# MarkTakken/kf2vecFSW

Measured on AMD Instinct MI355X. Metric: Gbases/s k-mer→.kf build at k=7; achieved HBM GB/s vs gfx950 peak, higher is better.
Workload: dtype u32

## Files before the change

kf2vecfsw_amd/counter.py:

```python
from __future__ import annotations

import ctypes
import dataclasses
import os
from typing import Sequence

import numpy as np
import torch

from . import _native as N

ALIGN = 16


def num_bins(k: int) -> int:
    return int(N.lib().kf_num_bins(k))


def tables(k: int) -> tuple[np.ndarray, np.ndarray]:
    nb = num_bins(k)
    code2col = np.empty(1 << (2 * k), dtype=np.uint32)
    col2rep = np.empty(nb, dtype=np.uint32)
    n = ctypes.c_uint64(0)
    N.check(N.lib().kf_tables(k, code2col.ctypes.data, col2rep.ctypes.data, ctypes.byref(n)), "kf_tables")
    assert n.value == nb
    return code2col, col2rep


def vocab_text(k: int) -> bytes:
    nb = num_bins(k)
    buf = np.empty(nb * (k + 1), dtype=np.uint8)
    w = ctypes.c_uint64(0)
    N.check(N.lib().kf_vocab_text(k, buf.ctypes.data, buf.size, ctypes.byref(w)), "kf_vocab_text")
    return buf[: w.value].tobytes()


def index_records(data: np.ndarray, fmt: int = N.KF_FMT_AUTO, base: int = 0) -> tuple[np.ndarray, int]:
    data = np.ascontiguousarray(data, dtype=np.uint8)
    cap = 64
    while True:
        out = np.empty(2 * cap, dtype=np.uint64)
        n = ctypes.c_uint64(0)
        f = ctypes.c_int(0)
        rc = N.lib().kf_index_records(data.ctypes.data, data.size, fmt, base, out.ctypes.data, cap,
                                      ctypes.byref(n), ctypes.byref(f))
        if rc == N.KF_ERANGE:
            cap = int(n.value)
            continue
        N.check(rc, "kf_index_records")
        return out[: 2 * n.value], int(f.value)


@dataclasses.dataclass
class HostBatch:
    data: torch.Tensor | None
    off: np.ndarray
    excl: np.ndarray | None
    names: list[str]
    dev_data: torch.Tensor | None = None
    dev_event: object = None
    fastq: bool = False

    @property
    def n(self) -> int:
        return len(self.off) - 1

    def seq_chars(self) -> int:
        d = self.data.numpy()
        nl = int(np.count_nonzero(d[: int(self.off[-1])] == 10))
        excl = self.excl if self.excl is not None else np.concatenate(
            [index_records(d[int(self.off[i]): int(self.off[i + 1])],
                           N.KF_FMT_FASTQ if self.fastq else N.KF_FMT_FASTA, int(self.off[i]))[0]
             for i in range(self.n)] or [np.zeros(0, np.uint64)])
        ex = int((excl[1::2] - excl[0::2]).sum()) if excl.size else 0
        return int(self.off[-1] - self.off[0]) - nl - ex


def _layout(sizes: Sequence[int]) -> np.ndarray:
    off = np.zeros(len(sizes) + 1, dtype=np.uint64)
    pos = 0
    for i, s in enumerate(sizes):
        off[i] = pos
        pos += (int(s) + ALIGN - 1) // ALIGN * ALIGN
    off[-1] = pos
    return off


def _alloc_host(nbytes: int, pin: bool) -> torch.Tensor:
    pin = pin and torch.cuda.is_available()
    return torch.empty(max(nbytes, ALIGN), dtype=torch.uint8, pin_memory=pin)


def pack_genomes(blobs: Sequence[bytes | np.ndarray], names: Sequence[str] | None = None,
                 fmt: int = N.KF_FMT_AUTO, pin: bool = True) -> HostBatch:
    sizes = [len(b) for b in blobs]
    off = _layout(sizes)
    data = _alloc_host(int(off[-1]), pin)
    d = data.numpy()
    d[: int(off[-1])] = 10
    excl = []
    for i, b in enumerate(blobs):
        a = np.frombuffer(b, dtype=np.uint8) if isinstance(b, (bytes, bytearray, memoryview)) else np.asarray(b, np.uint8)
        lo = int(off[i])
        d[lo: lo + a.size] = a
        iv, _ = index_records(d[lo: lo + a.size], fmt, lo)
        excl.append(iv)
    ex = np.concatenate(excl) if excl else np.zeros(0, np.uint64)
    return HostBatch(data, off, ex.astype(np.uint64), list(names) if names else [str(i) for i in range(len(blobs))])


def pack_files(paths: Sequence[str], names: Sequence[str] | None = None, fmt: int = N.KF_FMT_AUTO,
               pin: bool = True, threads: int = 8, pool=None, times: dict | None = None,
               buf: torch.Tensor | None = None, index: bool = True, piece: int = 1 << 20) -> HostBatch:
    from concurrent.futures import ThreadPoolExecutor
    import time
    t0 = time.perf_counter()
    sizes = [os.path.getsize(p) for p in paths]
    off = _layout(sizes)
    if buf is not None and buf.numel() >= max(int(off[-1]), ALIGN):
        data = buf[: max(int(off[-1]), ALIGN)]
    else:
        data = _alloc_host(int(off[-1]), pin)
    d = data.numpy()
    if times is not None:
        times["alloc_ms"] = round((time.perf_counter() - t0) * 1e3, 3)
    nthr = getattr(pool, "_max_workers", None) or max(1, int(threads))
    if paths:
        enc = [os.fsencode(p) for p in paths]
        arr = (ctypes.c_char_p * len(enc))(*enc)
        sz = np.asarray(sizes, dtype=np.uint64)
        N.check(N.lib().kf_read_files(arr, len(enc), sz.ctypes.data, off.ctypes.data, d.ctypes.data,
                                      int(piece), int(nthr)), "kf_read_files")

    def is_fastq(i: int) -> bool:
        return fmt == N.KF_FMT_FASTQ or (fmt == N.KF_FMT_AUTO and sizes[i] > 0 and d[int(off[i])] == ord("@"))

    def on_host(i: int) -> bool:
        return index or is_fastq(i)

    def host_index(i: int):
        lo, sz = int(off[i]), sizes[i]
        return index_records(d[lo: lo + sz], fmt, lo)[0] if on_host(i) else None

    if not any(on_host(i) for i in range(len(paths))):
        return HostBatch(data, off, None, list(names) if names else list(paths))
    if not index and all(is_fastq(i) or sizes[i] == 0 for i in range(len(paths))):
        return HostBatch(data, off, None, list(names) if names else list(paths), fastq=True)
    if pool is not None:
        excl = list(pool.map(host_index, range(len(paths))))
    elif threads > 1 and len(paths) > 1:
        with ThreadPoolExecutor(max_workers=min(threads, len(paths))) as ex:
            excl = list(ex.map(host_index, range(len(paths))))
    else:
        excl = [host_index(i) for i in range(len(paths))]
    if not index and all(e is None for e in excl):
        return HostBatch(data, off, None, list(names) if names else list(paths))
    excl = [e if e is not None else index_records(d[int(off[i]): int(off[i]) + sizes[i]], N.KF_FMT_FASTA,
                                                  int(off[i]))[0] for i, e in enumerate(excl)]
    ex = np.concatenate(excl) if excl else np.zeros(0, np.uint64)
    return HostBatch(data, off, ex.astype(np.uint64), list(names) if names else list(paths))


def pack_ranges(ranges: Sequence[tuple[str, int, int]], names: Sequence[str] | None = None, pin: bool = True,
                threads: int = 8, chunk: int = 64 << 20, index: bool = False, buf: torch.Tensor | None = None,
                fastq: bool = False) -> HostBatch:
    from concurrent.futures import ThreadPoolExecutor
    sizes = [e - a for _, a, e in ranges]
    off = _layout(sizes)
    if buf is not None and buf.numel() >= max(int(off[-1]), ALIGN):
        data = buf[: max(int(off[-1]), ALIGN)]
    else:
        data = _alloc_host(int(off[-1]), pin)
    d = data.numpy()
    for i, sz in enumerate(sizes):
        d[int(off[i]) + sz: int(off[i + 1])] = 10
    jobs = []
    for i, (p, a, e) in enumerate(ranges):
        for x in range(a, e, chunk):
            jobs.append((p, x, min(e, x + chunk), int(off[i]) + x - a))

    def read(job):
        p, x, y, dst = job
        fd = os.open(p, os.O_RDONLY)
        try:
            got = 0
            mv = memoryview(d[dst: dst + (y - x)])
            while got < y - x:
                r = os.preadv(fd, [mv[got:]], x + got)
                if r <= 0:
                    raise N.NativeError(f"short read on {p}")
                got += r
        finally:
            os.close(fd)

    with ThreadPoolExecutor(max_workers=max(1, int(threads))) as ex:
        list(ex.map(read, jobs))
        excl = None
        if index and not fastq:
            parts = list(ex.map(lambda i: index_records(d[int(off[i]): int(off[i]) + sizes[i]], N.KF_FMT_FASTA,
                                                        int(off[i]))[0], range(len(ranges))))
            excl = (np.concatenate(parts) if parts else np.zeros(0, np.uint64)).astype(np.uint64)
    return HostBatch(data, off, excl, list(names) if names else [f"{p}:{a}" for p, a, _ in ranges], fastq=fastq)


@dataclasses.dataclass
class DeviceBatch:
    data: torch.Tensor
    off: torch.Tensor
    excl: torch.Tensor
    n: int
    n_excl: int
    irregular: tuple = ()


def index_on_device(data: torch.Tensor, off: torch.Tensor, n: int, nbytes: int) -> tuple[torch.Tensor, int]:
    dev = data.device
    s = _stream_ptr(dev)
    nb = (nbytes + 4095) // 4096
    scratch = torch.empty(nb + 1, dtype=torch.int32, device=dev)
    npairs = torch.zeros(1, dtype=torch.int64, device=dev)
    cap = 64 * n + 4096
    while True:
        excl = torch.empty(max(2 * cap, 2), dtype=torch.int64, device=dev)
        N.check(N.lib().kf_index_fasta(data.data_ptr(), off.data_ptr(), n, nbytes, excl.data_ptr(), cap,
                                       npairs.data_ptr(), scratch.data_ptr(), nb + 1, s), "kf_index_fasta")
        m = int(npairs.item())
        if m <= cap:
            return excl[: 2 * m], m
        cap = m


def index_fastq_on_device(data: torch.Tensor, off: torch.Tensor, n: int, nbytes: int, status_out: list | None = None
                          ) -> tuple[torch.Tensor, int, bool]:
    dev = data.device
    s = _stream_ptr(dev)
    L = N.lib()
    cap_lines = nbytes // 32 + 4 * n + 4096
    cap_pairs = nbytes // 128 + 2 * n + 4096
    info = torch.empty(2 + (n + 1) // 2, dtype=torch.int64, device=dev)
    while True:
        need = int(L.kf_index_fastq_scratch_bytes(nbytes, n, cap_lines))
        scratch = torch.empty(max(need // 8, 1), dtype=torch.int64, device=dev)
        excl = torch.empty(max(2 * cap_pairs, 2), dtype=torch.int64, device=dev)
        N.check(L.kf_index_fastq(data.data_ptr(), off.data_ptr(), n, nbytes, excl.data_ptr(), cap_pairs, cap_lines,
                                 info.data_ptr(), info.data_ptr() + 16, scratch.data_ptr(), need, s), "kf_index_fastq")
        h = info.cpu().numpy()
        m, lines = int(h[0]), int(h[1])
        if lines > cap_lines:
            cap_lines, cap_pairs = lines, max(cap_pairs, lines // 4 + 2 * n + 1)
            continue
        if m > cap_pairs:
            cap_pairs = m
            continue
        status = h[2:].view(np.uint32)[:n]
        if (status == 2).any():
            raise N.NativeError("kf_index_fastq: genome offsets must be non-decreasing and end at or below the batch")
        if status_out is not None:
            status_out.append(status.copy())
        return excl[: 2 * m], m, not status.any()


INDEX_PATHS = {"fasta_device": 0, "fastq_device": 0, "fastq_host_fallback": 0}


def to_device(hb: HostBatch, device: torch.device | str = "cuda", fallback: bool = True) -> DeviceBatch:
    dev = torch.device(device)
    if hb.dev_data is not None:
        cur = torch.cuda.current_stream(dev)
        if hb.dev_event is not None:
            cur.wait_event(hb.dev_event)
        data = hb.dev_data
        data.record_stream(cur)
    else:
        data = hb.data.to(dev, non_blocking=True)
    if hb.excl is None:
        pin = hb.data is None or hb.data.is_pinned()
        off = torch.from_numpy(hb.off.view(np.int64))
        off = (off.pin_memory() if pin else off).to(dev, non_blocking=pin)
        nbytes = int(hb.off[-1])
        with torch.cuda.device(dev):
            if not hb.fastq:
                excl, m = index_on_device(data, off, hb.n, nbytes)
                INDEX_PATHS["fasta_device"] += 1
            else:
                st: list = []
                excl, m, regular = index_fastq_on_device(data, off, hb.n, nbytes, st)
                INDEX_PATHS["fastq_device" if regular or not fallback else "fastq_host_fallback"] += 1
                if not regular and not fallback:
                    return DeviceBatch(data, off, excl if m else torch.zeros(2, dtype=torch.int64, device=dev), hb.n, m,
                                       tuple(int(g) for g in np.flatnonzero(st[0])))
                if not regular:
                    d = data[:nbytes].cpu().numpy()
                    iv = np.concatenate([index_records(d[int(hb.off[i]): int(hb.off[i + 1])], N.KF_FMT_FASTQ,
                                                       int(hb.off[i]))[0] for i in range(hb.n)])
                    m = iv.size // 2
                    excl = torch.from_numpy(iv.view(np.int64)).to(dev)
        return DeviceBatch(data, off, excl if m else torch.zeros(2, dtype=torch.int64, device=dev), hb.n, m)
    ex = hb.excl if hb.excl.size else np.zeros(2, np.uint64)
    pin = hb.data is None or hb.data.is_pinned()
    n_off = (hb.off.size + 1) & ~1
    host = np.zeros(n_off + ex.size, np.int64)
    host[: hb.off.size] = hb.off.view(np.int64)
    host[n_off:] = ex.view(np.int64)
    small = torch.from_numpy(host)
    if pin:
        small = small.pin_memory()
    small = small.to(dev, non_blocking=pin)
    off, excl = small[: hb.off.size], small[n_off:]
    return DeviceBatch(data, off, excl, hb.n, hb.excl.size // 2)


def _stream_ptr(device: torch.device) -> int:
    return torch.cuda.current_stream(device).cuda_stream


def accumulate_rows(src: torch.Tensor, src_totals: torch.Tensor, seg: torch.Tensor, dst: torch.Tensor,
                    dst_totals: torch.Tensor, status: torch.Tensor, accumulate: bool = False,
                    stream: int | None = None) -> None:
    assert src.dtype == torch.int32 and dst.dtype == torch.int32 and src.is_contiguous() and dst.is_contiguous()
    assert src.dim() == 2 and dst.dim() == 2 and src.shape[1] == dst.shape[1]
    assert src_totals.dtype == torch.int64 and src_totals.shape == (src.shape[0],) and src_totals.is_contiguous()
    assert dst_totals.dtype == torch.int64 and dst_totals.shape == (dst.shape[0],) and dst_totals.is_contiguous()
    assert seg.dtype == torch.int32 and seg.shape == (dst.shape[0] + 1,) and seg.is_contiguous()
    assert status.dtype == torch.int32 and status.shape == (dst.shape[0],) and status.is_contiguous()
    s = _stream_ptr(dst.device) if stream is None else stream
    with torch.cuda.device(dst.device):
        N.check(N.lib().kf_rows_accumulate(src.data_ptr(), src_totals.data_ptr(), src.shape[0], seg.data_ptr(),
                                           dst.shape[0], dst.shape[1], dst.data_ptr(), dst_totals.data_ptr(),
                                           status.data_ptr(), N.KF_ACCUMULATE if accumulate else 0, s),
                "kf_rows_accumulate")


_DEV_TABLES: dict = {}


class KmerCounter:

    def __init__(self, k: int, device: torch.device | str = "cuda"):
        if not (N.KF_MIN_K <= k <= N.KF_MAX_K):
            raise ValueError(f"k={k} out of range [{N.KF_MIN_K}, {N.KF_MAX_K}]")
        self.k = k
        self.device = torch.device(device)
        if self.device.type != "cuda" or not torch.cuda.is_available():
            raise N.NativeError("KmerCounter needs a ROCm GPU (no CPU fallback)")
        self.nbins = num_bins(k)
        key = (k, self.device.index if self.device.index is not None else torch.cuda.current_device())
        if key not in _DEV_TABLES:
            c2c, c2r = tables(k)
            _DEV_TABLES[key] = (torch.from_numpy(c2c.view(np.int32)).to(self.device),
                                torch.from_numpy(c2r.view(np.int32)).to(self.device))
        self.code2col, self.col2rep = _DEV_TABLES[key]

    def launch_info(self) -> tuple[int, int, int]:
        g, b, l = ctypes.c_int(), ctypes.c_int(), ctypes.c_int()
        with torch.cuda.device(self.device):
            N.check(N.lib().kf_count_launch_info(self.k, ctypes.byref(g), ctypes.byref(b), ctypes.byref(l)),
                    "kf_count_launch_info")
        return g.value, b.value, l.value

    def reserve(self, max_genomes: int) -> None:
        with torch.cuda.device(self.device):
            N.check(N.lib().kf_workspace_reserve(self.k, int(max_genomes)), "kf_workspace_reserve")

    def alloc_out(self, n: int) -> tuple[torch.Tensor, torch.Tensor]:
        return (torch.empty((n, self.nbins), dtype=torch.int32, device=self.device),
                torch.empty(n, dtype=torch.int64, device=self.device))

    def count(self, db: DeviceBatch, counts: torch.Tensor | None = None, totals: torch.Tensor | None = None,
              accumulate: bool = False, stream: int | None = None) -> tuple[torch.Tensor, torch.Tensor]:
        if counts is None or totals is None:
            counts, totals = self.alloc_out(db.n)
        assert counts.shape == (db.n, self.nbins) and counts.dtype == torch.int32 and counts.is_contiguous()
        assert totals.shape == (db.n,) and totals.dtype == torch.int64
        assert db.data.data_ptr() % 16 == 0
        s = _stream_ptr(self.device) if stream is None else stream
        with torch.cuda.device(self.device):
            N.check(N.lib().kf_count_batch(
                db.data.data_ptr(), db.off.data_ptr(), db.n, db.excl.data_ptr() if db.n_excl else None,
                db.n_excl, self.code2col.data_ptr(), self.col2rep.data_ptr(), self.k,
                counts.data_ptr(), totals.data_ptr(), N.KF_ACCUMULATE if accumulate else 0, s), "kf_count_batch")
        return counts, totals


class SparseCounter:

    def __init__(self, k: int, device: torch.device | str = "cuda"):
        if not (N.KF_MIN_K <= k <= N.KF_SPARSE_MAX_K):
            raise ValueError(f"k={k} out of range [{N.KF_MIN_K}, {N.KF_SPARSE_MAX_K}]")
        self.k = k
        self.device = torch.device(device)
        if self.device.type != "cuda" or not torch.cuda.is_available():
            raise N.NativeError("SparseCounter needs a ROCm GPU (no CPU fallback)")
        self._work = None

    def workspace_bytes(self, batch_bytes: int, n: int) -> int:
        return int(N.lib().kf_sparse_workspace_bytes(self.k, int(batch_bytes), int(n)))

    def count(self, db: DeviceBatch, batch_bytes: int):
        batch_bytes = int(batch_bytes)
        need = self.workspace_bytes(batch_bytes, db.n)
        if self._work is None or self._work.numel() < need:
            self._work = None
            self._work = torch.empty(max(need, 256), dtype=torch.uint8, device=self.device)
        keys = torch.empty(max(batch_bytes, 1), dtype=torch.int64, device=self.device)
        counts = torch.empty(max(batch_bytes, 1), dtype=torch.int32, device=self.device)
        nuniq = torch.zeros(max(db.n, 1), dtype=torch.int64, device=self.device)
        s = _stream_ptr(self.device)
        with torch.cuda.device(self.device):
            N.check(N.lib().kf_sparse_count(
                db.data.data_ptr(), db.off.data_ptr(), db.n, batch_bytes,
                db.excl.data_ptr() if db.n_excl else None, db.n_excl, self.k,
                self._work.data_ptr(), self._work.numel(), keys.data_ptr(), counts.data_ptr(),
                nuniq.data_ptr(), s), "kf_sparse_count")
        return keys, counts, nuniq[: db.n]

    @staticmethod
    def nuniq_to_host(nuniq: torch.Tensor) -> np.ndarray:
        nu = nuniq.cpu().numpy()
        if nu.size and (nu == -1).any():
            raise N.NativeError("kf_sparse_count: genome offsets must be non-decreasing and end at or below "
                                "batch_bytes (nothing was counted)")
        if nu.size and (nu == -2).any():
            raise N.NativeError("kf_sparse_count: the sorted keys failed the device's order check")
        return nu

    def to_host(self, keys: torch.Tensor, counts: torch.Tensor, nuniq: torch.Tensor,
                off: np.ndarray) -> list[tuple[np.ndarray, np.ndarray]]:
        nu = self.nuniq_to_host(nuniq)
        if nu.size == 0 or int(nu.sum()) == 0:
            return [(np.zeros(0, np.uint64), np.zeros(0, np.uint32)) for _ in range(nu.size)]
        idx = torch.cat([torch.arange(int(off[g]), int(off[g]) + int(nu[g]), device=keys.device)
                         for g in range(nu.size)])
        hk = keys[idx].cpu().numpy().view(np.uint64)
        hc = counts[idx].cpu().numpy().view(np.uint32)
        out, pos = [], 0
        for g in range(nu.size):
            m = int(nu[g])
            out.append((hk[pos: pos + m], hc[pos: pos + m]))
            pos += m
        return out


def merge_tile() -> int:
    return int(N.lib().kf_sparse_merge_tile())


def merge_scratch_bytes(n_a: int, n_b: int) -> int:
    return int(N.lib().kf_sparse_merge_scratch_bytes(int(n_a), int(n_b)))


def merge_sorted(keys_a: torch.Tensor, counts_a: torch.Tensor, keys_b: torch.Tensor, counts_b: torch.Tensor,
                 stream: int | None = None):
    for k_, c_ in ((keys_a, counts_a), (keys_b, counts_b)):
        assert k_.dtype == torch.int64 and k_.dim() == 1 and k_.is_contiguous()
        assert c_.dtype in (torch.int32, torch.int64) and c_.shape == k_.shape and c_.is_contiguous()
        assert k_.device == keys_a.device and c_.device == keys_a.device
    dev = keys_a.device
    n_a, n_b = keys_a.numel(), keys_b.numel()
    keys = torch.empty(max(n_a + n_b, 1), dtype=torch.int64, device=dev)
    counts = torch.empty(max(n_a + n_b, 1), dtype=torch.int64, device=dev)
    n_out = torch.empty(1, dtype=torch.int64, device=dev)
    status = torch.empty(1, dtype=torch.int32, device=dev)
    need = merge_scratch_bytes(n_a, n_b)
    scratch = torch.empty(max(need // 8, 1), dtype=torch.int64, device=dev)
    s = _stream_ptr(dev) if stream is None else stream
    with torch.cuda.device(dev):
        N.check(N.lib().kf_sparse_merge(
            keys_a.data_ptr() if n_a else None, counts_a.data_ptr() if n_a else None,
            4 if counts_a.dtype == torch.int32 else 8, n_a,
            keys_b.data_ptr() if n_b else None, counts_b.data_ptr() if n_b else None,
            4 if counts_b.dtype == torch.int32 else 8, n_b,
            keys.data_ptr(), counts.data_ptr(), n_out.data_ptr(), status.data_ptr(), scratch.data_ptr(),
            8 * scratch.numel(), s), "kf_sparse_merge")
    return keys[: n_a + n_b], counts[: n_a + n_b], n_out, status


def merged_to_host(n_out: torch.Tensor, status: torch.Tensor) -> int:
    n, st = torch.cat([n_out, status.to(torch.int64)]).cpu().tolist()
    if st != 0:
        raise N.NativeError("kf_sparse_merge: an input list is not strictly ascending (nothing was merged)")
    return int(n)


def counts_to_numpy(counts: torch.Tensor) -> np.ndarray:
    return counts.cpu().numpy().view(np.uint32)


def features(counts: torch.Tensor, pseudocount: bool = False, raw_cnt: bool = False,
             scaler: float = 1.0) -> torch.Tensor:
    c = counts.to(torch.int64)
    c = torch.where(c < 0, c + (1 << 32), c)
    v = c.to(torch.float64)
    if pseudocount:
        v = v + 0.5
    if not raw_cnt:
        v = v / v.sum(dim=1, keepdim=True)
    return v * scaler if scaler != 1.0 else v


def chunk_features(counts: torch.Tensor, lo, n, scaler: float = 1.0, cap: int | None = None,
                   dtype: torch.dtype = torch.float32, out: torch.Tensor | None = None,
                   stream: int | None = None) -> torch.Tensor:
    assert counts.dtype in (torch.int16, torch.int32) and counts.dim() == 2 and counts.is_contiguous()
    assert dtype in (torch.float32, torch.float64)
    dev = counts.device
    if isinstance(lo, torch.Tensor) and lo.is_cuda:
        assert isinstance(n, torch.Tensor) and n.device == lo.device == dev and lo.shape == n.shape
        assert lo.dtype == n.dtype == torch.int64 and lo.is_contiguous() and n.is_contiguous()
        d_lo, d_n = lo, n
    else:
        def as_i64(x):
            x = np.asarray(x.cpu() if isinstance(x, torch.Tensor) else x)
            return x.view(np.int64) if x.dtype == np.uint64 else x.astype(np.int64)
        t = torch.from_numpy(np.stack([as_i64(lo).reshape(-1), as_i64(n).reshape(-1)]))
        d_lo, d_n = (t.pin_memory() if t.numel() else t).to(dev, non_blocking=True)
    ns, nbins = d_lo.numel(), counts.shape[1]
    if out is None:
        out = torch.empty((ns, nbins), dtype=dtype, device=dev)
    assert out.dtype == dtype and out.shape == (ns, nbins) and out.is_contiguous() and out.device == dev
    if ns == 0:
        return out
    status = torch.empty(1, dtype=torch.int32, device=dev)
    need = int(N.lib().kf_chunk_features_scratch_bytes(ns))
    work = torch.empty(need // 8, dtype=torch.int64, device=dev)
    s = _stream_ptr(dev) if stream is None else stream
    with torch.cuda.device(dev):
        N.check(N.lib().kf_chunk_features(
            counts.data_ptr() if counts.shape[0] else None, counts.element_size(), counts.shape[0], nbins,
            d_lo.data_ptr(), d_n.data_ptr(), ns, 0xFFFFFFFF if cap is None else int(cap), float(scaler),
# ... 220 lines not shown
```

kf2vecfsw_amd/csrc/kf_compact.h:

```cpp
#pragma once
#include "kf_scan.h"

namespace kf {
namespace {

constexpr int kCompactBlock = 256;
constexpr int kCompactPer = 16;
constexpr uint32_t kCompactSpan = kCompactBlock * kCompactPer;

__device__ __forceinline__ uint64_t compact_p0() {
    return (uint64_t)blockIdx.x * kCompactSpan + (uint64_t)threadIdx.x * kCompactPer;
}

template <typename T>
__device__ __forceinline__ void compact_count(uint32_t c, T* blk) {
    __shared__ uint32_t red[kCompactBlock / 64];
    const uint32_t all = block_sum<kCompactBlock / 64>(c, red);
    if (threadIdx.x == 0) blk[blockIdx.x] = all;
}

__device__ __forceinline__ uint64_t compact_first_slot(uint64_t base, uint32_t c) {
    __shared__ uint32_t wsum[kCompactBlock / 64];
    return base + block_excl_scan<kCompactBlock / 64>(c, wsum);
}

__global__ void __launch_bounds__(1024) compact_scan_kernel(uint32_t* blk, uint32_t nb, uint64_t* total64) {
    const uint32_t all = scan_with_carry(
        nb, [&](uint32_t i) { return blk[i]; }, [&](uint32_t i, uint32_t p) { blk[i] = p; });
    if (threadIdx.x == 0) {
        blk[nb] = all;
        if (total64) *total64 = all;
    }
}

}
}
```

kf2vecfsw_amd/csrc/kf_index.hip:

```cpp
#include <hip/hip_runtime.h>
#include <stdint.h>

#include "kf_compact.h"
#include "kf_internal.h"

namespace kf {
namespace {

constexpr int kIBlock = kCompactBlock;
constexpr int kIPer = kCompactPer;
constexpr uint32_t kISpan = kCompactSpan;

__device__ __forceinline__ uint32_t thread_heads(const uint8_t* bytes, uint64_t end, const uint64_t* goff, int n,
                                                 uint64_t p0) {
    uint32_t m = 0;
    if (p0 >= end) return 0;
    uint8_t prev = p0 > 0 ? bytes[p0 - 1] : (uint8_t)'\n';
    for (int q = 0; q < kIPer; ++q) {
        const uint64_t i = p0 + q;
        if (i >= end) break;
        const uint8_t c = bytes[i];
        if (c == '>') {
            bool start = prev == '\n' || i == 0;
            if (!start) {
                start = goff[last_at_or_before(n, i, [&](int g) { return goff[g]; })] == i;
            }
            if (start) m |= 1u << q;
        }
        prev = c;
    }
    return m;
}

__global__ void __launch_bounds__(kIBlock) idx_count_kernel(const uint8_t* bytes, uint64_t end, const uint64_t* goff,
                                                            int n, uint32_t* blk) {
    compact_count((uint32_t)__builtin_popcount(thread_heads(bytes, end, goff, n, compact_p0())), blk);
}

__global__ void __launch_bounds__(kIBlock) idx_scatter_kernel(const uint8_t* bytes, uint64_t end, const uint64_t* goff,
                                                              int n, const uint32_t* blk, uint64_t* excl,
                                                              uint64_t cap) {
    const uint64_t p0 = compact_p0();
    uint32_t m = thread_heads(bytes, end, goff, n, p0);
    uint64_t u = compact_first_slot(blk[blockIdx.x], (uint32_t)__builtin_popcount(m));
    while (m) {
        const int q = __builtin_ctz(m);
        m &= m - 1;
        const uint64_t j = p0 + (uint64_t)q;
        if (u < cap) {
            const uint64_t ge = goff[last_at_or_before(n, j, [&](int g) { return goff[g]; }) + 1];
            uint64_t e = j;
            while (e < ge && bytes[e] != '\n') ++e;
            excl[2 * u] = j;
            excl[2 * u + 1] = e;
        }
        ++u;
    }
}

constexpr uint32_t kQLevel = kScanLevel;
constexpr uint64_t kQMaxEntries = kScanMaxEntries;
constexpr auto fq_scan_level_kernel = scan_level_kernel<uint64_t>;

struct FqLayout {
    uint64_t nb, nb1, nb2;
    uint64_t ng1, ng2;
    uint64_t blk, blk1, blk2, g_nl, g_lines, g_end, g_pairs, g_pairs1, g_pairs2, nlpos, words;
};

inline uint64_t div_up(uint64_t a, uint64_t b) { return (a + b - 1) / b; }

inline FqLayout fq_layout(uint64_t batch_bytes, uint64_t n_genomes, uint64_t cap_lines) {
    FqLayout L;
    L.nb = div_up(batch_bytes, kISpan);
    L.nb1 = div_up(L.nb, kQLevel);
    L.nb2 = div_up(L.nb1, kQLevel);
    L.ng1 = div_up(n_genomes, kQLevel);
    L.ng2 = div_up(L.ng1, kQLevel);
    uint64_t w = 0;
    L.blk = w, w += L.nb;
    L.blk1 = w, w += L.nb1;
    L.blk2 = w, w += L.nb2;
    L.g_nl = w, w += n_genomes;
    L.g_lines = w, w += n_genomes;
    L.g_end = w, w += n_genomes;
    L.g_pairs = w, w += n_genomes;
    L.g_pairs1 = w, w += L.ng1;
    L.g_pairs2 = w, w += L.ng2;
    L.nlpos = w, w += cap_lines;
    L.words = w;
    return L;
}

__device__ __forceinline__ uint32_t nl_bits(uint32_t w) {
    const uint32_t x = w ^ 0x0A0A0A0Au;
    const uint32_t z = ~(((x & 0x7F7F7F7Fu) + 0x7F7F7F7Fu) | x | 0x7F7F7F7Fu);
    return (((z >> 7) * 0x00204081u) >> 21) & 0xFu;
}

__device__ __forceinline__ uint32_t thread_newlines(const uint8_t* bytes, uint64_t end, uint64_t p0) {
    if (p0 >= end) return 0;
    const uint4 v = *reinterpret_cast<const uint4*>(bytes + p0);
    uint32_t m = nl_bits(v.x) | nl_bits(v.y) << 4 | nl_bits(v.z) << 8 | nl_bits(v.w) << 12;
    if (end - p0 < kIPer) m &= (1u << (uint32_t)(end - p0)) - 1u;
    return m;
}

__global__ void __launch_bounds__(kIBlock) fq_count_kernel(const uint8_t* bytes, uint64_t end, uint64_t* blk) {
    compact_count((uint32_t)__builtin_popcount(thread_newlines(bytes, end, compact_p0())), blk);
}

__global__ void __launch_bounds__(kIBlock) fq_scatter_kernel(const uint8_t* bytes, uint64_t end, const uint64_t* blk,
                                                             const uint64_t* blk1, const uint64_t* blk2,
                                                             uint64_t* nlpos, uint64_t cap_lines) {
    const uint64_t p0 = compact_p0();
    uint32_t m = thread_newlines(bytes, end, p0);
    uint64_t u = compact_first_slot(scanned(blk, blk1, blk2, blockIdx.x), (uint32_t)__builtin_popcount(m));
    while (m) {
        const int q = __builtin_ctz(m);
        m &= m - 1;
        if (u < cap_lines) nlpos[u] = p0 + (uint64_t)q;
        ++u;
    }
}

__device__ __forceinline__ uint64_t first_at_or_after(const uint64_t* pos, uint64_t n, uint64_t x) {
    uint64_t lo = 0, hi = n;
    while (lo < hi) {
        const uint64_t mid = lo + ((hi - lo) >> 1);
        if (pos[mid] < x) lo = mid + 1;
        else hi = mid;
    }
    return lo;
}

__global__ void __launch_bounds__(kIBlock) fq_genome_kernel(const uint64_t* goff, int n, uint64_t end,
                                                            const uint64_t* nlpos, const uint64_t* n_lines,
                                                            uint64_t cap_lines, uint64_t* g_nl, uint64_t* g_lines,
                                                            uint64_t* g_end, uint64_t* g_pairs, uint32_t* status) {
    const uint64_t g = (uint64_t)blockIdx.x * kIBlock + threadIdx.x;
    if (g >= (uint64_t)n) return;
    const uint64_t tot = *n_lines, a = goff[g], b = goff[g + 1];
    uint64_t first = 0, lines = 0, cend = a;
    if (tot <= cap_lines) {
        if (b < a || b > end) {
            status[g] = 2;
        } else {
            first = first_at_or_after(nlpos, tot, a);
            const uint64_t last = first_at_or_after(nlpos, tot, b);
            uint64_t lo = first, hi = last;
            while (lo < hi) {
                const uint64_t mid = lo + ((hi - lo) >> 1);
                if (nlpos[mid] + (last - mid) == b) hi = mid;
                else lo = mid + 1;
            }
            cend = b - (last - lo);
            if (cend > a) lines = (lo - first) + 1;
        }
    }
    g_nl[g] = first;
    g_lines[g] = lines;
    g_end[g] = cend;
    g_pairs[g] = lines ? 1 + (lines + 1) / 4 : 0;
}

__global__ void __launch_bounds__(kIBlock) fq_pair_kernel(const uint8_t* bytes, const uint64_t* goff, int n,
                                                          const uint64_t* nlpos, const uint64_t* n_lines,
                                                          uint64_t cap_lines, const uint64_t* g_nl,
                                                          const uint64_t* g_lines, const uint64_t* g_end,
                                                          const uint64_t* g_pairs, const uint64_t* g_pairs1,
                                                          const uint64_t* g_pairs2, const uint64_t* n_pairs,
                                                          uint64_t* excl, uint64_t cap_pairs, uint32_t* status) {
    const uint64_t q = (uint64_t)blockIdx.x * kIBlock + threadIdx.x;
    if (q >= cap_pairs || q >= *n_pairs || *n_lines > cap_lines) return;
    const uint64_t g = (uint64_t)last_at_or_before(
        n, q, [&](int m) { return scanned(g_pairs, g_pairs1, g_pairs2, (uint64_t)m); });
    const uint64_t r = q - scanned(g_pairs, g_pairs1, g_pairs2, g);
    const uint64_t lines = g_lines[g], a = goff[g], cend = g_end[g];
    const uint64_t* nl = nlpos + g_nl[g];
    if (lines == 0 || r >= 1 + (lines + 1) / 4) return;
    auto start_of = [&](uint64_t j) { return j == 0 ? a : nl[j - 1] + 1; };
    auto end_of = [&](uint64_t j) { return j + 1 < lines ? nl[j] : cend; };
    uint64_t s, e;
    if (r == 0) {
        s = a;
        e = end_of(0);
    } else {
        const uint64_t plus = 4 * r - 2, to = plus + 2 < lines ? plus + 2 : lines - 1;
        s = start_of(plus);
        e = end_of(to);
    }
    excl[2 * q] = s;
    excl[2 * q + 1] = e;
    const uint64_t j0 = 4 * r;
    if (j0 >= lines) return;
    bool bad;
    uint64_t len_seq = 0;
    {
        const uint64_t s0 = start_of(j0), e0 = end_of(j0);
        bad = !(e0 > s0 && bytes[s0] == '@');
    }
    if (j0 + 1 < lines) {
        const uint64_t s1 = start_of(j0 + 1);
        len_seq = end_of(j0 + 1) - s1;
        bad |= len_seq > 0 && bytes[s1] == '+';
    }
    if (j0 + 2 < lines) {
        const uint64_t s2 = start_of(j0 + 2);
        bad |= !(end_of(j0 + 2) > s2 && bytes[s2] == '+');
    }
    if (j0 + 3 < lines) {
        const uint64_t len_qual = end_of(j0 + 3) - start_of(j0 + 3);
        bad |= len_seq == 0 ? len_qual != 0 : len_qual < len_seq;
    }
    if (bad) status[g] = 1;
}

}
}

using namespace kf;

extern "C" int kf_index_fasta(const uint8_t* d_bytes, const uint64_t* d_goff, int32_t n_genomes, uint64_t batch_bytes,
                              uint64_t* d_excl, uint64_t cap_pairs, uint64_t* d_n_pairs, uint32_t* d_scratch,
                              uint64_t scratch_words, void* stream) {
    if (n_genomes < 0) return kf_fail(KF_EINVAL, "n_genomes < 0");
    if (!d_n_pairs) return kf_fail(KF_EINVAL, "null device pointer");
    hipStream_t s = (hipStream_t)stream;
    if (n_genomes == 0 || batch_bytes == 0) {
        if (hipMemsetAsync(d_n_pairs, 0, 8, s) != hipSuccess) return kf_fail(KF_EHIP, "memset failed");
        return KF_OK;
    }
    if (!d_bytes || !d_goff || !d_scratch || (cap_pairs && !d_excl)) return kf_fail(KF_EINVAL, "null device pointer");
    const uint64_t nb = (batch_bytes + kISpan - 1) / kISpan;
    if (nb >= (1ull << 31)) return kf_fail(KF_EINVAL, "batch too large");
    if (scratch_words < nb + 1)
        return kf_fail(KF_ERANGE, "scratch needs %llu words", (unsigned long long)(nb + 1));
    hipLaunchKernelGGL(idx_count_kernel, dim3((uint32_t)nb), dim3(kIBlock), 0, s, d_bytes, batch_bytes, d_goff,
                       n_genomes, d_scratch);
    hipLaunchKernelGGL(compact_scan_kernel, dim3(1), dim3(1024), 0, s, d_scratch, (uint32_t)nb, d_n_pairs);
    hipLaunchKernelGGL(idx_scatter_kernel, dim3((uint32_t)nb), dim3(kIBlock), 0, s, d_bytes, batch_bytes, d_goff,
                       n_genomes, d_scratch, d_excl, cap_pairs);
    if (hipGetLastError() != hipSuccess) return kf_fail(KF_EHIP, "record index launch failed");
    return KF_OK;
}

extern "C" uint64_t kf_index_fastq_scratch_bytes(uint64_t batch_bytes, int32_t n_genomes, uint64_t cap_lines) {
    if (n_genomes < 0) return 0;
    return 8 * fq_layout(batch_bytes, (uint64_t)n_genomes, cap_lines).words;
}

extern "C" int kf_index_fastq(const uint8_t* d_bytes, const uint64_t* d_goff, int32_t n_genomes, uint64_t batch_bytes,
                              uint64_t* d_excl, uint64_t cap_pairs, uint64_t cap_lines, uint64_t* d_n,
                              uint32_t* d_status, void* d_scratch, uint64_t scratch_bytes, void* stream) {
    if (n_genomes < 0) return kf_fail(KF_EINVAL, "n_genomes < 0");
    if (!d_n) return kf_fail(KF_EINVAL, "null device pointer (d_n)");
    if (n_genomes > 0 && !d_status) return kf_fail(KF_EINVAL, "null device pointer (d_status)");
    hipStream_t s = (hipStream_t)stream;
    if (n_genomes == 0 || batch_bytes == 0) {
        if (hipMemsetAsync(d_n, 0, 16, s) != hipSuccess ||
            (n_genomes && hipMemsetAsync(d_status, 0, 4 * (size_t)n_genomes, s) != hipSuccess))
            return kf_fail(KF_EHIP, "memset failed");
        return KF_OK;
    }
    if (!d_bytes || !d_goff || !d_scratch || (cap_pairs && !d_excl)) return kf_fail(KF_EINVAL, "null device pointer");
    if (((uintptr_t)d_bytes & 15) || ((uintptr_t)d_scratch & 7))
        return kf_fail(KF_EINVAL, "d_bytes must be 16-byte and d_scratch 8-byte aligned");
    const FqLayout L = fq_layout(batch_bytes, (uint64_t)n_genomes, cap_lines);
    if (L.nb > kQMaxEntries) return kf_fail(KF_EINVAL, "batch too large");
    if ((uint64_t)n_genomes > kQMaxEntries) return kf_fail(KF_EINVAL, "too many genomes");
    if (cap_pairs >= (1ull << 31) * kIBlock) return kf_fail(KF_EINVAL, "cap_pairs too large");
    if (scratch_bytes < 8 * L.words)
        return kf_fail(KF_ERANGE, "scratch needs %llu bytes", (unsigned long long)(8 * L.words));
    uint64_t* w = (uint64_t*)d_scratch;
    if (hipMemsetAsync(d_status, 0, 4 * (size_t)n_genomes, s) != hipSuccess) return kf_fail(KF_EHIP, "memset failed");
    hipLaunchKernelGGL(fq_count_kernel, dim3((uint32_t)L.nb), dim3(kIBlock), 0, s, d_bytes, batch_bytes, w + L.blk);
    hipLaunchKernelGGL(fq_scan_level_kernel, dim3((uint32_t)L.nb1), dim3(kQLevel), 0, s, w + L.blk, L.nb, w + L.blk1);
    hipLaunchKernelGGL(fq_scan_level_kernel, dim3((uint32_t)L.nb2), dim3(kQLevel), 0, s, w + L.blk1, L.nb1,
                       w + L.blk2);
    hipLaunchKernelGGL(fq_scan_level_kernel, dim3(1), dim3(kQLevel), 0, s, w + L.blk2, L.nb2, d_n + 1);
    hipLaunchKernelGGL(fq_scatter_kernel, dim3((uint32_t)L.nb), dim3(kIBlock), 0, s, d_bytes, batch_bytes, w + L.blk,
                       w + L.blk1, w + L.blk2, w + L.nlpos, cap_lines);
    const uint32_t gb = (uint32_t)div_up((uint64_t)n_genomes, kIBlock);
    hipLaunchKernelGGL(fq_genome_kernel, dim3(gb), dim3(kIBlock), 0, s, d_goff, n_genomes, batch_bytes, w + L.nlpos,
                       d_n + 1, cap_lines, w + L.g_nl, w + L.g_lines, w + L.g_end, w + L.g_pairs, d_status);
    hipLaunchKernelGGL(fq_scan_level_kernel, dim3((uint32_t)L.ng1), dim3(kQLevel), 0, s, w + L.g_pairs,
                       (uint64_t)n_genomes, w + L.g_pairs1);
    hipLaunchKernelGGL(fq_scan_level_kernel, dim3((uint32_t)L.ng2), dim3(kQLevel), 0, s, w + L.g_pairs1, L.ng1,
                       w + L.g_pairs2);
    hipLaunchKernelGGL(fq_scan_level_kernel, dim3(1), dim3(kQLevel), 0, s, w + L.g_pairs2, L.ng2, d_n);
    if (cap_pairs)
        hipLaunchKernelGGL(fq_pair_kernel, dim3((uint32_t)div_up(cap_pairs, kIBlock)), dim3(kIBlock), 0, s, d_bytes,
                           d_goff, n_genomes, w + L.nlpos, d_n + 1, cap_lines, w + L.g_nl, w + L.g_lines, w + L.g_end,
                           w + L.g_pairs, w + L.g_pairs1, w + L.g_pairs2, d_n, d_excl, cap_pairs, d_status);
    if (hipGetLastError() != hipSuccess) return kf_fail(KF_EHIP, "FASTQ index launch failed");
    return KF_OK;
}
```

kf2vecfsw_amd/csrc/kf_scan.h:

```cpp
#pragma once
#include <hip/hip_runtime.h>
#include <stdint.h>

namespace kf {

typedef __attribute__((address_space(3))) uint32_t lds_u32;
__device__ __forceinline__ void lds_add(uint32_t a, uint32_t v) {
    __hip_atomic_fetch_add((lds_u32*)(uintptr_t)a, v, __ATOMIC_RELAXED, __HIP_MEMORY_SCOPE_WORKGROUP);
}
__device__ __forceinline__ uint32_t lds_add_rtn(uint32_t a, uint32_t v) {
    return __hip_atomic_fetch_add((lds_u32*)(uintptr_t)a, v, __ATOMIC_RELAXED, __HIP_MEMORY_SCOPE_WORKGROUP);
}

__device__ __forceinline__ void lds_barrier() { asm volatile("s_waitcnt lgkmcnt(0)\n\ts_barrier" ::: "memory"); }

__device__ __forceinline__ uint32_t wave_incl_scan(uint32_t v) {
    v += (uint32_t)__builtin_amdgcn_update_dpp(0, (int)v, 0x111, 0xF, 0xF, false);
    v += (uint32_t)__builtin_amdgcn_update_dpp(0, (int)v, 0x112, 0xF, 0xF, false);
    v += (uint32_t)__builtin_amdgcn_update_dpp(0, (int)v, 0x114, 0xF, 0xF, false);
    v += (uint32_t)__builtin_amdgcn_update_dpp(0, (int)v, 0x118, 0xF, 0xF, false);
    v += (uint32_t)__builtin_amdgcn_update_dpp(0, (int)v, 0x142, 0xA, 0xF, false);
    v += (uint32_t)__builtin_amdgcn_update_dpp(0, (int)v, 0x143, 0xC, 0xF, false);
    return v;
}
__device__ __forceinline__ uint64_t wave_incl_scan(uint64_t v) {
    const int lane = threadIdx.x & 63;
    for (int d = 1; d < 64; d <<= 1) {
        const uint64_t o = __shfl_up((unsigned long long)v, d, 64);
        if (lane >= d) v += o;
    }
    return v;
}

template <int NW, bool LDSB = false, typename T>
__device__ __forceinline__ T block_excl_scan(T v, T* wsum, T* total = nullptr) {
    const int lane = threadIdx.x & 63, w = threadIdx.x >> 6;
    const T inc = wave_incl_scan(v);
    if (lane == 63) wsum[w] = inc;
    if (LDSB) lds_barrier();
    else __syncthreads();
    T before = 0, all = 0;
#pragma unroll
    for (int x = 0; x < NW; ++x) {
        const T s = wsum[x];
        before += x < w ? s : T(0);
        all += s;
    }
    if (total) *total = all;
    if (LDSB) lds_barrier();
    else __syncthreads();
    return before + inc - v;
}

template <int NW>
__device__ __forceinline__ uint32_t block_sum(uint32_t v, uint32_t* red) {
    const uint32_t inc = wave_incl_scan(v);
    if ((threadIdx.x & 63) == 63) red[threadIdx.x >> 6] = inc;
    __syncthreads();
    uint32_t all = 0;
#pragma unroll
    for (int x = 0; x < NW; ++x) all += red[x];
    return all;
}

template <typename Load, typename Store>
__device__ __forceinline__ uint32_t scan_with_carry(uint32_t n, Load load, Store store) {
    __shared__ uint32_t wsum[16];
    uint32_t carry = 0;
    for (uint32_t base = 0; base < n; base += 1024) {
        const uint32_t i = base + threadIdx.x;
        uint32_t tot;
        const uint32_t ex = block_excl_scan<16>(i < n ? (uint32_t)load(i) : 0u, wsum, &tot);
        if (i < n) store(i, carry + ex);
        carry += tot;
    }
    return carry;
}

constexpr uint32_t kScanLevel = 1024;
constexpr uint64_t kScanMaxEntries = (uint64_t)kScanLevel * kScanLevel * kScanLevel;

namespace {
template <typename T>
__global__ void __launch_bounds__(kScanLevel) scan_level_kernel(T* v, uint64_t n, T* sums) {
    __shared__ T wsum[kScanLevel / 64];
    const uint64_t i = (uint64_t)blockIdx.x * kScanLevel + threadIdx.x;
    T all;
    const T ex = block_excl_scan<kScanLevel / 64>(i < n ? v[i] : T(0), wsum, &all);
    if (i < n) v[i] = ex;
    if (threadIdx.x == 0) sums[blockIdx.x] = all;
}
}

__device__ __forceinline__ uint64_t scanned(const uint64_t* v, const uint64_t* s1, const uint64_t* s2, uint64_t i) {
    return v[i] + s1[i >> 10] + s2[i >> 20];
}

template <typename X, typename Key>
__device__ __forceinline__ int last_at_or_before(int n, X x, Key key) {
    int lo = 0, hi = n;
    while (hi - lo > 1) {
        const int m = (lo + hi) >> 1;
        if (key(m) <= x) lo = m;
        else hi = m;
    }
    return lo;
}

}
```

Baseline: 5853.

## Replace FASTA index count/scan/scatter with single-pass decoupled look-back kernel

Replaces the three-kernel FASTA header index (count, single-block scan, scatter) with one kernel. Each block takes a 128 KiB tile through an atomic ticket, builds '>' and newline bitmasks in LDS with vector loads, and gets its output offset by decoupled look-back over per-tile status words. This cuts the input reads from two to one, drops two launches, and replaces the byte-by-byte line-end search with bitmask lookups. In exchange it adds a memset, a spin-wait with a poll bound that can fail and report an error, and a new 16-byte alignment requirement on the input.

After: 5853, median of 2. No clear change (+0.0%).

```diff
diff --git a/kf2vecfsw_amd/counter.py b/kf2vecfsw_amd/counter.py
--- a/kf2vecfsw_amd/counter.py
+++ b/kf2vecfsw_amd/counter.py
@@ -225,6 +225,8 @@
         N.check(N.lib().kf_index_fasta(data.data_ptr(), off.data_ptr(), n, nbytes, excl.data_ptr(), cap,
                                        npairs.data_ptr(), scratch.data_ptr(), nb + 1, s), "kf_index_fasta")
         m = int(npairs.item())
+        if m < 0:
+            raise N.NativeError("kf_index_fasta: the index did not complete (a tile's look-back wait ran out)")
         if m <= cap:
             return excl[: 2 * m], m
         cap = m
diff --git a/kf2vecfsw_amd/csrc/kf_compact.h b/kf2vecfsw_amd/csrc/kf_compact.h
--- a/kf2vecfsw_amd/csrc/kf_compact.h
+++ b/kf2vecfsw_amd/csrc/kf_compact.h
@@ -24,7 +24,8 @@
     return base + block_excl_scan<kCompactBlock / 64>(c, wsum);
 }
 
-__global__ void __launch_bounds__(1024) compact_scan_kernel(uint32_t* blk, uint32_t nb, uint64_t* total64) {
+[[maybe_unused]] __global__ void __launch_bounds__(1024) compact_scan_kernel(uint32_t* blk, uint32_t nb,
+                                                                             uint64_t* total64) {
     const uint32_t all = scan_with_carry(
         nb, [&](uint32_t i) { return blk[i]; }, [&](uint32_t i, uint32_t p) { blk[i] = p; });
     if (threadIdx.x == 0) {
@@ -33,5 +34,66 @@
     }
 }
 
+struct OnePass {
+    uint32_t* ctl;
+    uint64_t* status;
+    uint32_t ntiles;
+};
+
+inline uint64_t onepass_words(const uint32_t* d_scratch, uint64_t ntiles) {
+    return 4 + (((uintptr_t)d_scratch >> 2) & 1) + 2 * ntiles;
+}
+inline OnePass onepass_carve(uint32_t* d_scratch, uint32_t ntiles) {
+    return OnePass{d_scratch, (uint64_t*)(d_scratch + 4 + (((uintptr_t)d_scratch >> 2) & 1)), ntiles};
+}
+
+__device__ __forceinline__ uint32_t onepass_tile(const OnePass& P) {
+    __shared__ uint32_t tile;
+    if (P.ntiles == 1) return 0;
+    if (threadIdx.x == 0) tile = atomicAdd(P.ctl, 1u);
+    __syncthreads();
+    return tile;
+}
+
+__device__ __forceinline__ uint64_t onepass_first(const OnePass& P, uint32_t t, uint32_t c, uint64_t* incl,
+                                                  bool* lost) {
+    __shared__ uint32_t wsum[kCompactBlock / 64];
+    __shared__ uint64_t base[2];
+    uint32_t all;
+    const uint32_t ex = block_excl_scan<kCompactBlock / 64>(c, wsum, &all);
+    *lost = false;
+    if (P.ntiles == 1) {
+        *incl = all;
+        return ex;
+    }
+    if (threadIdx.x < 64) {
+        bool l;
+        const uint64_t b = tile_lookback(P.status, t, all, &l);
+        if (threadIdx.x == 0) base[0] = b, base[1] = l;
+    }
+    __syncthreads();
+    *lost = base[1] != 0;
+    *incl = base[0] + all;
+    return base[0] + ex;
+}
+
+__device__ __forceinline__ void onepass_finish(const OnePass& P, uint32_t t, uint64_t incl, bool lost,
+                                               uint64_t* total64) {
+    if (threadIdx.x != 0) return;
+    if (P.ntiles == 1) {
+        *total64 = incl;
+        return;
+    }
+    if (t == P.ntiles - 1) {
+        __hip_atomic_store(total64, lost ? ~0ull : incl, __ATOMIC_RELAXED, __HIP_MEMORY_SCOPE_AGENT);
+        asm volatile("s_waitcnt vmcnt(0)" ::: "memory");
+        if (__hip_atomic_fetch_or(P.ctl + 1, 1u, __ATOMIC_RELAXED, __HIP_MEMORY_SCOPE_AGENT) & 2u)
+            __hip_atomic_store(total64, ~0ull, __ATOMIC_RELAXED, __HIP_MEMORY_SCOPE_AGENT);
+    } else if (lost) {
+        if (__hip_atomic_fetch_or(P.ctl + 1, 2u, __ATOMIC_RELAXED, __HIP_MEMORY_SCOPE_AGENT) & 1u)
+            __hip_atomic_store(total64, ~0ull, __ATOMIC_RELAXED, __HIP_MEMORY_SCOPE_AGENT);
+    }
+}
+
 }
 }
diff --git a/kf2vecfsw_amd/csrc/kf_index.hip b/kf2vecfsw_amd/csrc/kf_index.hip
--- a/kf2vecfsw_amd/csrc/kf_index.hip
+++ b/kf2vecfsw_amd/csrc/kf_index.hip
@@ -11,51 +11,108 @@
 constexpr int kIPer = kCompactPer;
 constexpr uint32_t kISpan = kCompactSpan;
 
-__device__ __forceinline__ uint32_t thread_heads(const uint8_t* bytes, uint64_t end, const uint64_t* goff, int n,
-                                                 uint64_t p0) {
-    uint32_t m = 0;
-    if (p0 >= end) return 0;
-    uint8_t prev = p0 > 0 ? bytes[p0 - 1] : (uint8_t)'\n';
-    for (int q = 0; q < kIPer; ++q) {
-        const uint64_t i = p0 + q;
-        if (i >= end) break;
-        const uint8_t c = bytes[i];
-        if (c == '>') {
-            bool start = prev == '\n' || i == 0;
-            if (!start) {
-                start = goff[last_at_or_before(n, i, [&](int g) { return goff[g]; })] == i;
+constexpr uint32_t kITile = 131072;
+constexpr int kIRounds = kITile / kISpan;
+constexpr uint32_t kIUnits = kITile / kIPer;
+constexpr int kIBatch = kIRounds < 8 ? kIRounds : 8;
+static_assert((kITile & (kITile - 1)) == 0 && kITile <= 131072, "tile: a power of two, at most 128 KiB");
+static_assert(kIRounds >= 8, "tile: at least 8 spans");
+
+typedef uint32_t v4u_t __attribute__((ext_vector_type(4)));
+
+__device__ __forceinline__ uint32_t eq_bits(uint32_t w, uint32_t c4) {
+    const uint32_t x = w ^ c4;
+    const uint32_t z = ~(((x & 0x7F7F7F7Fu) + 0x7F7F7F7Fu) | x | 0x7F7F7F7Fu);
+    return (((z >> 7) * 0x00204081u) >> 21) & 0xFu;
+}
+__device__ __forceinline__ uint32_t eq_bits16(v4u_t v, uint32_t c4) {
+    return eq_bits(v.x, c4) | eq_bits(v.y, c4) << 4 | eq_bits(v.z, c4) << 8 | eq_bits(v.w, c4) << 12;
+}
+constexpr uint32_t kNl4 = 0x0A0A0A0Au, kGt4 = 0x3E3E3E3Eu;
+
+__device__ __forceinline__ uint64_t line_end_from(const uint8_t* bytes, uint64_t from, uint64_t lim) {
+    for (uint64_t e = from; e < lim; e += kIPer) {
+        const uint32_t m = eq_bits16(*reinterpret_cast<const v4u_t*>(bytes + e), kNl4);
+        if (m) return min(e + (uint64_t)__builtin_ctz(m), lim);
+    }
+    return lim;
+}
+
+__global__ void __launch_bounds__(kIBlock) idx_onepass_kernel(const uint8_t* bytes, uint64_t end, const uint64_t* goff,
+                                                              int n, OnePass P, uint64_t* excl, uint64_t cap,
+                                                              uint64_t* n_pairs) {
+    __shared__ uint16_t gtm[kIUnits], nlm[kIUnits];
+    __shared__ uint32_t prev_nl;
+    const uint32_t tid = threadIdx.x;
+    const uint32_t t = onepass_tile(P);
+    const uint64_t t0 = (uint64_t)t * kITile;
+    if (tid == 0) prev_nl = t0 == 0 || bytes[t0 - 1] == '\n';
+    for (int r0 = 0; r0 < kIRounds; r0 += kIBatch) {
+        v4u_t v[kIBatch];
+#pragma unroll
+        for (int r = 0; r < kIBatch; ++r) {
+            const uint64_t p = t0 + (uint64_t)(r0 + r) * kISpan + tid * kIPer;
+            const v4u_t* src = reinterpret_cast<const v4u_t*>(bytes + p);
+            v[r] = v4u_t{0, 0, 0, 0};
+            if (p < end) v[r] = *src;
+        }
+#pragma unroll
+        for (int r = 0; r < kIBatch; ++r) {
+            const uint64_t p = t0 + (uint64_t)(r0 + r) * kISpan + tid * kIPer;
+            const uint32_t live = p < end && end - p < kIPer ? (1u << (uint32_t)(end - p)) - 1u : 0xFFFFu;
+            gtm[(r0 + r) * kIBlock + tid] = (uint16_t)(eq_bits16(v[r], kGt4) & live);
+            nlm[(r0 + r) * kIBlock + tid] = (uint16_t)(eq_bits16(v[r], kNl4) & live);
+        }
+    }
+    __syncthreads();
+    const uint32_t u0 = tid * kIRounds;
+    uint32_t c = 0;
+    uint32_t carry = u0 ? nlm[u0 - 1] >> 15 : prev_nl;
+#pragma unroll
+    for (int i = 0; i < kIRounds; ++i) {
+        const uint32_t gt = gtm[u0 + i], nl = nlm[u0 + i];
+        uint32_t s = gt & ((nl << 1) | carry);
+        uint32_t rest = gt & ~s;
+        carry = nl >> 15;
+        while (rest) {
+            const int q = __builtin_ctz(rest);
+            rest &= rest - 1;
+            const uint64_t j = t0 + (uint64_t)(u0 + i) * kIPer + q;
+            if (goff[last_at_or_before(n, j, [&](int g) { return goff[g]; })] == j) s |= 1u << q;
+        }
+        c += __builtin_popcount(s);
+        if (s != gt) gtm[u0 + i] = (uint16_t)s;
+    }
+    uint64_t incl;
+    bool lost;
+    uint64_t u = onepass_first(P, t, c, &incl, &lost);
+    if (c && !lost && u < cap) {
+        int g = -1;
+#pragma unroll 1
+        for (int i = 0; i < kIRounds; ++i) {
+            uint32_t s = gtm[u0 + i];
+            while (s && u < cap) {
+                const int q = __builtin_ctz(s);
+                s &= s - 1;
+                const uint64_t j = t0 + (uint64_t)(u0 + i) * kIPer + q;
+                if (g < 0) g = last_at_or_before(n, j, [&](int x) { return goff[x]; });
+                else if (g + 1 < n && goff[g + 1] <= j) {
+                    const int g1 = g + 1;
+                    g = g1 + last_at_or_before(n - g1, j, [&](int x) { return goff[g1 + x]; });
+                }
+                const uint64_t lim = min(goff[g + 1], end);
+                uint32_t w = u0 + i;
+                uint32_t nl = nlm[w] & ~((2u << q) - 1u);
+                while (!nl && ++w < kIUnits) nl = nlm[w];
+                const uint64_t e = nl ? t0 + (uint64_t)w * kIPer + __builtin_ctz(nl)
+                                      : line_end_from(bytes, t0 + kITile, lim);
+                excl[2 * u] = j;
+                excl[2 * u + 1] = max(j, min(e, lim));
+                ++u;
             }
-            if (start) m |= 1u << q;
-        }
-        prev = c;
-    }
-    return m;
-}
-
-__global__ void __launch_bounds__(kIBlock) idx_count_kernel(const uint8_t* bytes, uint64_t end, const uint64_t* goff,
-                                                            int n, uint32_t* blk) {
-    compact_count((uint32_t)__builtin_popcount(thread_heads(bytes, end, goff, n, compact_p0())), blk);
-}
-
-__global__ void __launch_bounds__(kIBlock) idx_scatter_kernel(const uint8_t* bytes, uint64_t end, const uint64_t* goff,
-                                                              int n, const uint32_t* blk, uint64_t* excl,
-                                                              uint64_t cap) {
-    const uint64_t p0 = compact_p0();
-    uint32_t m = thread_heads(bytes, end, goff, n, p0);
-    uint64_t u = compact_first_slot(blk[blockIdx.x], (uint32_t)__builtin_popcount(m));
-    while (m) {
-        const int q = __builtin_ctz(m);
-        m &= m - 1;
-        const uint64_t j = p0 + (uint64_t)q;
-        if (u < cap) {
-            const uint64_t ge = goff[last_at_or_before(n, j, [&](int g) { return goff[g]; }) + 1];
-            uint64_t e = j;
-            while (e < ge && bytes[e] != '\n') ++e;
-            excl[2 * u] = j;
-            excl[2 * u + 1] = e;
-        }
-        ++u;
-    }
+        }
+    }
+    onepass_finish(P, t, incl, lost, n_pairs);
 }
 
 constexpr uint32_t kQLevel = kScanLevel;
@@ -92,11 +149,7 @@
     return L;
 }
 
-__device__ __forceinline__ uint32_t nl_bits(uint32_t w) {
-    const uint32_t x = w ^ 0x0A0A0A0Au;
-    const uint32_t z = ~(((x & 0x7F7F7F7Fu) + 0x7F7F7F7Fu) | x | 0x7F7F7F7Fu);
-    return (((z >> 7) * 0x00204081u) >> 21) & 0xFu;
-}
+__device__ __forceinline__ uint32_t nl_bits(uint32_t w) { return eq_bits(w, kNl4); }
 
 __device__ __forceinline__ uint32_t thread_newlines(const uint8_t* bytes, uint64_t end, uint64_t p0) {
     if (p0 >= end) return 0;
@@ -232,15 +285,20 @@
         return KF_OK;
     }
     if (!d_bytes || !d_goff || !d_scratch || (cap_pairs && !d_excl)) return kf_fail(KF_EINVAL, "null device pointer");
+    if (((uintptr_t)d_bytes & 15) || ((uintptr_t)d_scratch & 3))
+        return kf_fail(KF_EINVAL, "d_bytes must be 16-byte and d_scratch 4-byte aligned");
     const uint64_t nb = (batch_bytes + kISpan - 1) / kISpan;
     if (nb >= (1ull << 31)) return kf_fail(KF_EINVAL, "batch too large");
     if (scratch_words < nb + 1)
         return kf_fail(KF_ERANGE, "scratch needs %llu words", (unsigned long long)(nb + 1));
-    hipLaunchKernelGGL(idx_count_kernel, dim3((uint32_t)nb), dim3(kIBlock), 0, s, d_bytes, batch_bytes, d_goff,
-                       n_genomes, d_scratch);
-    hipLaunchKernelGGL(compact_scan_kernel, dim3(1), dim3(1024), 0, s, d_scratch, (uint32_t)nb, d_n_pairs);
-    hipLaunchKernelGGL(idx_scatter_kernel, dim3((uint32_t)nb), dim3(kIBlock), 0, s, d_bytes, batch_bytes, d_goff,
-                       n_genomes, d_scratch, d_excl, cap_pairs);
+    const uint32_t ntiles = (uint32_t)((batch_bytes + kITile - 1) / kITile);
+    if (ntiles > 1) {
+        const uint64_t words = onepass_words(d_scratch, ntiles);
+        if (words > nb + 1) return kf_fail(KF_ERANGE, "index scratch layout: %llu words", (unsigned long long)words);
+        if (hipMemsetAsync(d_scratch, 0, 4 * words, s) != hipSuccess) return kf_fail(KF_EHIP, "memset failed");
+    }
+    hipLaunchKernelGGL(idx_onepass_kernel, dim3(ntiles), dim3(kIBlock), 0, s, d_bytes, batch_bytes, d_goff, n_genomes,
+                       onepass_carve(d_scratch, ntiles), d_excl, cap_pairs, d_n_pairs);
     if (hipGetLastError() != hipSuccess) return kf_fail(KF_EHIP, "record index launch failed");
     return KF_OK;
 }
diff --git a/kf2vecfsw_amd/csrc/kf_scan.h b/kf2vecfsw_amd/csrc/kf_scan.h
--- a/kf2vecfsw_amd/csrc/kf_scan.h
+++ b/kf2vecfsw_amd/csrc/kf_scan.h
@@ -96,6 +96,71 @@
     return v[i] + s1[i >> 10] + s2[i >> 20];
 }
 
+constexpr uint64_t kTileAgg = 1, kTileIncl = 2, kTileLost = 3;
+constexpr uint64_t kTileCount = (1ull << 62) - 1;
+constexpr uint32_t kTilePollBound = 1u << 22;
+constexpr int kTileWindows = 4;
+
+__device__ __forceinline__ void tile_publish(uint64_t* w, uint64_t flag, uint64_t v) {
+    __hip_atomic_store(w, (flag << 62) | v, __ATOMIC_RELAXED, __HIP_MEMORY_SCOPE_AGENT);
+}
+
+__device__ __forceinline__ uint64_t wave_sum(uint64_t v) {
+    for (int d = 32; d; d >>= 1) v += __shfl_xor((unsigned long long)v, d, 64);
+    return v;
+}
+
+__device__ __forceinline__ uint64_t tile_lookback(uint64_t* status, uint32_t t, uint64_t tot, bool* lost) {
+    const int lane = threadIdx.x & 63;
+    *lost = false;
+    if (t == 0) {
+        if (lane == 0) tile_publish(status, kTileIncl, tot);
+        return 0;
+    }
+    if (lane == 0) tile_publish(status + t, kTileAgg, tot);
+    uint64_t before = 0;
+    uint32_t polls = 0;
+    bool bad = false;
+    int64_t hi = (int64_t)t - 1;
+    for (bool done = false; !done;) {
+        uint64_t w[kTileWindows];
+#pragma unroll
+        for (int k = 0; k < kTileWindows; ++k) {
+            const int64_t j = hi - 64 * k - lane;
+            w[k] = j >= 0 ? __hip_atomic_load(status + j, __ATOMIC_RELAXED, __HIP_MEMORY_SCOPE_AGENT)
+                          : kTileIncl << 62;
+        }
+        uint64_t add = 0;
+        bool wait = false;
+#pragma unroll
+        for (int k = 0; k < kTileWindows; ++k) {
+            if (done || wait) continue;
+            const uint64_t f = w[k] >> 62;
+            const uint64_t stop = __ballot(f >= kTileIncl);
+            const uint64_t need = stop ? (((stop & (0 - stop)) << 1) - 1) : ~0ull;
+            if (__ballot(f == 0) & need) {
+                wait = true;
+                continue;
+            }
+            add += ((need >> lane) & 1) ? (w[k] & kTileCount) : 0ull;
+            bad = (__ballot(f == kTileLost) & need) != 0;
+            done = stop != 0;
+            hi -= 64;
+        }
+        before += wave_sum(add);
+        if (wait) {
+            if (++polls > kTilePollBound) {
+                bad = true;
+                break;
+            }
+            __builtin_amdgcn_s_sleep(1);
+        }
+    }
+    if (lane == 0) tile_publish(status + t, bad ? kTileLost : kTileIncl, (before + tot) & kTileCount);
+    *lost = bad;
+    return before;
+}
+
 template <typename X, typename Key>
 __device__ __forceinline__ int last_at_or_before(int n, X x, Key key) {
     int lo = 0, hi = n;
```
